# NVIDIA-AI-IOT/redtail

Measured on AMD Instinct MI355X. Metric: stereo pairs/sec, ResNet18-2D 1257x369, higher is better.
Workload: dtype f32

## Files before the change

### redtail_amd/csrc/kernels/common.hip.h

```cpp
#pragma once
#include <hip/hip_runtime.h>
#include <stdint.h>

namespace rt {

typedef float f32x4 __attribute__((ext_vector_type(4)));
typedef float f32x16 __attribute__((ext_vector_type(16)));
typedef _Float16 f16x2 __attribute__((ext_vector_type(2)));
typedef _Float16 f16x4 __attribute__((ext_vector_type(4)));
typedef _Float16 f16x8 __attribute__((ext_vector_type(8)));

constexpr int kWave = 64;

#ifndef RT_WAVES_PER_EU
#define RT_WAVES_PER_EU(n) __attribute__((amdgpu_waves_per_eu(n, n)))
#endif

__host__ __device__ static inline int64_t cdiv(int64_t a, int64_t b) { return (a + b - 1) / b; }
__host__ __device__ static inline int round_up(int a, int b) { return (a + b - 1) / b * b; }

__device__ static __forceinline__ float elu1(float x) { return x > 0.f ? x : expf(x) - 1.f; }
__device__ static __forceinline__ float sigmoid1(float x) { return 1.f / (1.f + expf(-x)); }

template <int ACT>
// ... 15 lines not shown

typedef __amdgpu_buffer_rsrc_t buf_rsrc;
constexpr unsigned kBufOOB = 0x80000000u;
constexpr unsigned kBufSpan = 0x80000000u;
__device__ static __forceinline__ buf_rsrc make_buf(const void* base, bool valid = true) {
    return __builtin_amdgcn_make_buffer_rsrc(const_cast<void*>(base), 0, valid ? kBufSpan : 0u, 0x00020000);
}
__device__ static __forceinline__ float buf_load(buf_rsrc r, unsigned voff, unsigned soff) {
    return __builtin_bit_cast(float, __builtin_amdgcn_raw_buffer_load_b32(r, voff, soff, 0));
}
__device__ static __forceinline__ f32x4 buf_load4(buf_rsrc r, unsigned voff, unsigned soff) {
    return __builtin_bit_cast(f32x4, __builtin_amdgcn_raw_buffer_load_b128(r, voff, soff, 0));
}
typedef float f32x2_t __attribute__((ext_vector_type(2)));
typedef unsigned u32x2_t __attribute__((ext_vector_type(2)));
typedef unsigned u32x4_t __attribute__((ext_vector_type(4)));
__device__ static __forceinline__ f32x2_t buf_load2(buf_rsrc r, unsigned voff, unsigned soff) {
    return __builtin_bit_cast(f32x2_t, __builtin_amdgcn_raw_buffer_load_b64(r, voff, soff, 0));
}
__device__ static __forceinline__ void buf_store2(f32x2_t v, buf_rsrc r, unsigned voff, unsigned soff) {
    __builtin_amdgcn_raw_buffer_store_b64(__builtin_bit_cast(u32x2_t, v), r, voff, soff, 0);
}
__device__ static __forceinline__ void buf_store4(f32x4 v, buf_rsrc r, unsigned voff, unsigned soff) {
    __builtin_amdgcn_raw_buffer_store_b128(__builtin_bit_cast(u32x4_t, v), r, voff + soff, 0u, 0);
}
__device__ static __forceinline__ void buf_store(float v, buf_rsrc r, unsigned voff, unsigned soff) {
    __builtin_amdgcn_raw_buffer_store_b32(__builtin_bit_cast(unsigned, v), r, voff, soff, 0);
}

#ifndef RT_LDS_PTR
#define RT_LDS_PTR(p) ((__attribute__((address_space(3))) void*)(p))
#endif

#ifdef HIPEMU
__device__ static __forceinline__ void wait_vmem() {}
template <int N> __device__ static __forceinline__ void wait_vmem_but() {}
static inline void sload2_i32(const void* base, int off0, int off1, int& a, int& b) {
    a = *reinterpret_cast<const int*>(static_cast<const char*>(base) + off0);
    b = *reinterpret_cast<const int*>(static_cast<const char*>(base) + off1);
}
static inline void sload2_i64(const void* base, int off0, int off1, long long& a, long long& b) {
    a = *reinterpret_cast<const long long*>(static_cast<const char*>(base) + off0);
    b = *reinterpret_cast<const long long*>(static_cast<const char*>(base) + off1);
}
__device__ static __forceinline__ void lds_barrier() { __syncthreads(); }
__device__ static __forceinline__ void wave_lds_sync() { (void)__shfl(0.f, 0); }
__device__ static __forceinline__ unsigned pack_f16(float lo, float hi) {
    return (unsigned)__builtin_bit_cast(unsigned short, (_Float16)lo) | ((unsigned)__builtin_bit_cast(unsigned short, (_Float16)hi) << 16);
}
#else
__device__ static __forceinline__ void sload2_i32(const void* base, int off0, int off1, int& a, int& b) {
    asm volatile("s_load_dword %0, %2, %3\n\ts_load_dword %1, %2, %4\n\ts_waitcnt lgkmcnt(0)" : "=&s"(a), "=&s"(b) : "s"(base), "s"(off0), "s"(off1) : "memory");
}
__device__ static __forceinline__ void sload2_i64(const void* base, int off0, int off1, long long& a, long long& b) {
    asm volatile("s_load_dwordx2 %0, %2, %3\n\ts_load_dwordx2 %1, %2, %4\n\ts_waitcnt lgkmcnt(0)" : "=&s"(a), "=&s"(b) : "s"(base), "s"(off0), "s"(off1) : "memory");
}
__device__ static __forceinline__ void wait_vmem() { asm volatile("s_waitcnt vmcnt(0)" ::: "memory"); }
template <int N> __device__ static __forceinline__ void wait_vmem_but() { asm volatile("s_waitcnt vmcnt(%0)" ::"n"(N) : "memory"); }
__device__ static __forceinline__ void lds_barrier() { asm volatile("s_waitcnt lgkmcnt(0)\n\ts_barrier" ::: "memory"); }
__device__ static __forceinline__ void wave_lds_sync() {
    __builtin_amdgcn_fence(__ATOMIC_RELEASE, "wavefront");
    __builtin_amdgcn_wave_barrier();
    __builtin_amdgcn_fence(__ATOMIC_ACQUIRE, "wavefront");
}
__device__ static __forceinline__ unsigned pack_f16(float lo, float hi) {
    unsigned r;
// ... 38 lines not shown
```

### redtail_amd/csrc/kernels/conv_mfma.hip.h

```cpp
#pragma once
#include <type_traits>
#include "common.hip.h"

namespace rt {

struct ZSlice {
    int pad_y, pad_x;
    int Ho, Wo;
    int ch_row;
    unsigned tap_mask;
    int64_t y_off;
    int64_t w_off;
    int64_t r_off;
    int64_t r_off_il8;
    int64_t y_off_il8;
    int64_t r_off_il4;
};

struct ConvArgs {
    const float* x;
    float* y;
    const float* w;
    const float* bias;
    const float* resid;
    unsigned long long* dbg;
    const float* zeros;
    const ZSlice* zs;
    const int* ch_off;
    int CinPad;
    int Cout;
    int Hi, Wi;
    int x_pitch;
    int Ho, Wo;
    int pad_y, pad_x;
    int nz;
    int tiles_x;
    int act;
    int xcd_order;
    int64_t x_bstride;
    int64_t y_bstride;
    int64_t y_cstride;
    int64_t y_zstride;
    int64_t y_off;
    int y_ystride, y_xstride;
    int64_t r_cstride;
    int64_t r_bstride;
    int r_il8;
    int batch;
    int cin_real;
    int64_t x_cstride;
    const int* ch_shift;
    int w_exact;
    int z_inner;
    int nb_inner;
    int dw_seg, dw_nseg, dw_cpc, dw_ntiles;
    const float* x2;
    int x2_from;
};

#define RT_WG_TILE_NB(p, tile, zi, n, nblk)                                                         \
    int tile = blockIdx.x;                                                                          \
    if ((p).xcd_order) {                           \
        const int nwg_ = gridDim.x, q_ = nwg_ >> 3, r_ = nwg_ & 7;                                  \
        const int xcd_ = blockIdx.x & 7, idx_ = blockIdx.x >> 3;                                    \
        tile = (xcd_ < r_ ? xcd_ * (q_ + 1) : r_ * (q_ + 1) + (xcd_ - r_) * q_) + idx_;             \
    }                                                                                               \
    int nblk = blockIdx.y;                                                                          \
    if ((p).nb_inner > 0) { nblk = tile % (p).nb_inner; tile /= (p).nb_inner; }                     \
    int zi, n;                                                                                      \
    if ((p).z_inner) { zi = tile % (p).nz; tile /= (p).nz; n = blockIdx.z; }                        \
    else { zi = blockIdx.z % (p).nz; n = blockIdx.z / (p).nz; }
#define RT_WG_TILE(p, tile, zi, n) RT_WG_TILE_NB(p, tile, zi, n, nblk_unused_); (void)nblk_unused_;

#ifdef RT_KERNEL_TIMING
#define RT_TSTAMP() do { if (dbgp && tid == 0 && dbi < 16) dbgp[dbi++] = __builtin_amdgcn_s_memtime(); } while (0)
#else
#define RT_TSTAMP() do { } while (0)
#endif

#ifndef RT_ABLATE
#define RT_ABLATE 0
#endif
constexpr bool kAblGather = (RT_ABLATE & 1) != 0;
constexpr bool kAblWLoad = (RT_ABLATE & 2) != 0;
constexpr bool kAblLdsWr = (RT_ABLATE & 4) != 0;
constexpr bool kAblBarrier = (RT_ABLATE & 8) != 0;
constexpr bool kAblResid = (RT_ABLATE & 16) != 0;
constexpr bool kAblStore = (RT_ABLATE & 32) != 0;
constexpr bool kAblLdsRd = (RT_ABLATE & 64) != 0;
constexpr bool kAblXform = (RT_ABLATE & 128) != 0;
// ... 399 lines not shown
```

### redtail_amd/csrc/kernels/conv_rbd.hip.h

```cpp
#pragma once
#include "conv_split.hip.h"

namespace rt {

struct S3RBDCfg {
    static constexpr int NW = 8, NT = 512;
    static constexpr int SW = 30, XCOL = 34, TCOL = 32, STEP = 4;
    static constexpr int RX = 16, RT = 10;
    static constexpr int GXB = XCOL * 32, XROWB = 4 * GXB;
    static constexpr int GTB = TCOL * 32, TROWB = 4 * GTB;
    static constexpr int BSLOTS = STEP * XROWB / 16;
    static constexpr int NPIECE = BSLOTS / 64;
    static constexpr int PPW = (NPIECE + NW - 1) / NW;
    static constexpr int WL_SLOTS = 18 * 64;
    static_assert(BSLOTS % 64 == 0, "a batch is a whole number of DMA pieces");
};

__device__ static __forceinline__ int rbd_swz(int p) { return ((p >> 3) & 1) * 16; }

__device__ static __forceinline__ void rbd_dma16(buf_rsrc rs, void* lds_wave_base, unsigned voff, unsigned soff) {
#ifdef HIPEMU
    __builtin_amdgcn_raw_ptr_buffer_load_lds(rs, lds_wave_base, 16, voff, soff, 0, 0);
#else
    const unsigned m = (unsigned)(uintptr_t)(__attribute__((address_space(3))) char*)(lds_wave_base);
    asm volatile("s_mov_b32 m0, %0\n\ts_nop 0\n\tbuffer_load_dwordx4 %1, %2, %3 offen lds" ::"s"(m), "v"(voff), "s"(rs), "s"(soff) : "memory", "m0");
#endif
}

template <int J>
__device__ static __forceinline__ float rbd_join(unsigned hi2, unsigned lo2, float inv) {
#ifdef HIPEMU
    const _Float16 h = __builtin_bit_cast(_Float16, (unsigned short)(hi2 >> (16 * J))), l = __builtin_bit_cast(_Float16, (unsigned short)(lo2 >> (16 * J)));
    return fmaf((float)l, inv, (float)h);
#else
    float r;
    if (J == 0) asm("v_fma_mix_f32 %0, %1, %2, %3 op_sel:[0,0,0] op_sel_hi:[1,0,1]" : "=v"(r) : "v"(lo2), "v"(inv), "v"(hi2));
    else asm("v_fma_mix_f32 %0, %1, %2, %3 op_sel:[1,0,1] op_sel_hi:[1,0,1]" : "=v"(r) : "v"(lo2), "v"(inv), "v"(hi2));
    return r;
#endif
}

__device__ static __forceinline__ float rbd_elu(float v) { return elu_fast(v); }

#ifndef RT_RBD_PRIO
#define RT_RBD_PRIO 0
#endif
#ifndef RT_RBD_ABL
#define RT_RBD_ABL 0
#endif
#ifndef RT_RBD_PF
#define RT_RBD_PF 1
#endif

template <bool Y_SPLIT>
__global__ void __launch_bounds__(512) RT_WAVES_PER_EU(2) conv_s3rbd_kernel(RBArgs a) {
    using Cfg = S3RBDCfg;
    const ConvArgs& p = a.c;
    constexpr int RX = Cfg::RX, RT = Cfg::RT, GXB = Cfg::GXB, XROWB = Cfg::XROWB, GTB = Cfg::GTB, TROWB = Cfg::TROWB, PPW = Cfg::PPW;

    __shared__ __attribute__((aligned(1024))) char sX[RX * XROWB];
    __shared__ __attribute__((aligned(1024))) char sT[(RT + 2) * TROWB];
// ... 21 lines not shown
        tile = (xcd < r ? xcd * (q + 1) : r * (q + 1) + (xcd - r) * q) + idx;
    }
    const int H = p.Hi, W = p.Wi;
    const int c0 = (tile % p.tiles_x) * Cfg::SW;
    const int y0 = (tile / p.tiles_x) * a.seg;
    const int y1 = y0 + a.seg < H ? y0 + a.seg : H;
    const int t0 = y0 - 1;
    const int n = blockIdx.z;
    const int nstep = (y1 - t0 + 4) / 4 + 1;
    const int last1 = (y1 - t0) / 4;
    const int row_hi = (y1 + 1 < H - 1 ? y1 + 1 : H - 1);

    const buf_rsrc rs_x = make_buf(elem_ptr(p.x, (int64_t)n * p.x_bstride, 4));
    const unsigned gsb_x = (unsigned)p.x_cstride * 32u, rowb_x = (unsigned)p.x_pitch * 32u;
    unsigned xvo[PPW];
    int xnb[PPW];
#pragma unroll
    for (int j = 0; j < PPW; j++) {
        const int k = (wv + 8 * j) * 64 + lane;
        const int r = k / (XROWB / 16), rem = k - r * (XROWB / 16);
        const int g = rem / (GXB / 16), rem2 = rem - g * (GXB / 16);
        const int px = rem2 >> 1, lo = (rem2 & 1) != ((px >> 3) & 1);
        const int ix = c0 - 2 + px;
        const bool valid = wv + 8 * j < Cfg::NPIECE && ix >= 0 && ix < W;
        xvo[j] = valid ? (unsigned)g * gsb_x + (unsigned)(t0 + 1 + r) * rowb_x + (unsigned)ix * 32u + (lo ? 16u : 0u) : kBufOOB;
        const int d = row_hi - (t0 + 1 + r);
        xnb[j] = valid && d >= 0 ? (d >> 2) + 1 : 0;
    }
    auto issue_batch = [&](int b) __attribute__((always_inline)) {
        const unsigned so = (unsigned)(4 * b) * rowb_x;
        char* dst = sX + ((4 * b + 4) & (RX - 1)) * XROWB;
#pragma unroll
        for (int j = 0; j < PPW; j++)
            if (wv + 8 * j < Cfg::NPIECE) rbd_dma16(rs_x, dst + (wv + 8 * j) * 1024, b < xnb[j] ? xvo[j] : kBufOOB, so);
    };

#pragma unroll
    for (int j = 0; j < PPW; j++) {
        if (wv + 8 * j >= Cfg::NPIECE) continue;
        const int r = ((wv + 8 * j) * 64 + lane) / (XROWB / 16);
        const bool ok = xvo[j] != kBufOOB && r >= 2 && t0 - 3 + r >= 0;
        rbd_dma16(rs_x, sX + (wv + 8 * j) * 1024, ok ? xvo[j] - 4u * rowb_x : kBufOOB, 0u);
    }
    issue_batch(0);
    {
        const buf_rsrc rs_w = make_buf(is1 ? a.w1 : p.w);
#pragma unroll
        for (int jj = 0; jj < 9; jj++) {
            const int pw = wr + 4 * jj, t = pw >> 1;
            char* dst = (pw & 1) ? reinterpret_cast<char*>(sWl + (is1 ? 0 : Cfg::WL_SLOTS)) + t * 1024 : sT + (is1 ? 0 : Cfg::WL_SLOTS * 16) + t * 1024;
            rbd_dma16(rs_w, dst, (unsigned)lane * 16u, (unsigned)pw * 1024u);
        }
    }
    f32x16 biasv;
    {
        const float* bsrc = is1 ? a.bias1 : p.bias;
#pragma unroll
        for (int q = 0; q < 4; q++) {
            const f32x4 bv = *reinterpret_cast<const f32x4*>(bsrc + 16 * (q >> 1) + 8 * kg + 4 * (q & 1));
#pragma unroll
            for (int e = 0; e < 4; e++) biasv[4 * q + e] = bv[e];
        }
    }
    RBD_STAMP(1);
    wait_vmem();
#ifndef HIPEMU
    asm volatile("" : "+v"(biasv));
#endif
    __syncthreads();
    f16x8 wh[18];
    {
        const f32x4* whs = reinterpret_cast<const f32x4*>(sT) + (is1 ? 0 : Cfg::WL_SLOTS) + lane;
#pragma unroll
        for (int t = 0; t < 18; t++) wh[t] = __builtin_bit_cast(f16x8, whs[t * 64]);
    }
    __syncthreads();
    RBD_STAMP(2);

    const f32x4* wlp = sWl + (is1 ? 0 : Cfg::WL_SLOTS) + lane;
    int bo_h[3], bo_l[3];
#pragma unroll
    for (int s = 0; s < 3; s++) {
        bo_h[s] = kg * (is1 ? GXB : GTB) + (l31 + s) * 32 + rbd_swz(l31 + s);
        bo_l[s] = bo_h[s] ^ 16;
// ... 185 lines not shown
```

### redtail_amd/csrc/kernels/conv_rbh.hip.h

```cpp
#pragma once
#include "conv_rbd.hip.h"

namespace rt {

struct F16RBDCfg {
    static constexpr int NW = 8, NT = 512;
    static constexpr int SW = 30, XCOL = 36, TCOL = 32, STEP = 4;
    static constexpr int RX = 20, RT = 10;
    static constexpr int GXB = XCOL * 16, XROWB = 4 * GXB;
    static constexpr int GTB = TCOL * 16, TROWB = 4 * GTB;
    static constexpr int BSLOTS = STEP * XROWB / 16;
    static constexpr int NPIECE = BSLOTS / 64;
    static constexpr int PPW = (NPIECE + 3) / 4;
    static constexpr int W_SLOTS = 18 * 64;
    static_assert(BSLOTS % 64 == 0, "a batch is a whole number of DMA pieces");
};

template <int J>
__device__ static __forceinline__ float rbh_add16(unsigned h2, float b) {
#ifdef HIPEMU
    return b + (float)__builtin_bit_cast(_Float16, (unsigned short)(h2 >> (16 * J)));
#else
    float r;
    if (J == 0) asm("v_fma_mix_f32 %0, %1, 1.0, %2 op_sel:[0,0,0] op_sel_hi:[1,0,0]" : "=v"(r) : "v"(h2), "v"(b));
// ... 25 lines not shown
        const int xcd = blockIdx.x & 7, idx = blockIdx.x >> 3;
        tile = (xcd < r ? xcd * (q + 1) : r * (q + 1) + (xcd - r) * q) + idx;
    }
    const int H = p.Hi, W = p.Wi;
    const int c0 = (tile % p.tiles_x) * Cfg::SW;
    const int y0 = (tile / p.tiles_x) * a.seg;
    const int y1 = y0 + a.seg < H ? y0 + a.seg : H;
    const int t0 = y0 - 1;
    const int n = blockIdx.z;
    const int nstep = (y1 - t0 + 4) / 4 + 1;
    const int last1 = (y1 - t0) / 4;
    const int row_hi = (y1 + 1 < H - 1 ? y1 + 1 : H - 1);

    const buf_rsrc rs_x = make_buf(elem_ptr(p.x, (int64_t)n * p.x_bstride, ES));
    const unsigned gsb_x = (unsigned)p.x_cstride * 16u, rowb_x = (unsigned)p.x_pitch * 16u;
    unsigned xvo[PPW];
    int xnb[PPW];
#pragma unroll
    for (int j = 0; j < PPW; j++) {
        const int k = (wr + 4 * j) * 64 + lane;
        const int r = k / (XROWB / 16), rem = k - r * (XROWB / 16);
        const int g = rem / Cfg::XCOL, px = rem - g * Cfg::XCOL;
        const int ix = c0 - 2 + px;
        const bool valid = is1 && wr + 4 * j < Cfg::NPIECE && px < 34 && ix >= 0 && ix < W;
        xvo[j] = valid ? (unsigned)g * gsb_x + (unsigned)(t0 + 1 + r) * rowb_x + (unsigned)ix * 16u : kBufOOB;
        const int d = row_hi - (t0 + 1 + r);
        xnb[j] = valid && d >= 0 ? (d >> 2) + 1 : 0;
    }
    auto issue_batch = [&](int b) __attribute__((always_inline)) {
        const unsigned so = (unsigned)(4 * b) * rowb_x;
        char* dst = sX + ((4 * b + 4) % RX) * XROWB;
#pragma unroll
        for (int j = 0; j < PPW; j++)
            if (wr + 4 * j < Cfg::NPIECE) rbd_dma16(rs_x, dst + (wr + 4 * j) * 1024, b < xnb[j] ? xvo[j] : kBufOOB, so);
    };

    if (is1) {
#pragma unroll
        for (int j = 0; j < PPW; j++) {
            if (wr + 4 * j >= Cfg::NPIECE) continue;
            const int r = ((wr + 4 * j) * 64 + lane) / (XROWB / 16);
            const bool ok = xvo[j] != kBufOOB && r >= 2 && t0 - 3 + r >= 0;
            rbd_dma16(rs_x, sX + (wr + 4 * j) * 1024, ok ? xvo[j] - 4u * rowb_x : kBufOOB, 0u);
        }
        issue_batch(0);
        issue_batch(1);
    }
    {
        const buf_rsrc rs_w = make_buf(is1 ? a.w1 : p.w);
        for (int t = wr; t < 18; t += 4)
            rbd_dma16(rs_w, (is1 ? sT : sX + 12 * XROWB) + t * 1024, (unsigned)lane * 16u, (unsigned)t * 1024u);
    }
    f32x16 biasv;
    {
        const float* bsrc = is1 ? a.bias1 : p.bias;
#pragma unroll
        for (int q = 0; q < 4; q++) {
            const f32x4 bv = *reinterpret_cast<const f32x4*>(bsrc + 16 * (q >> 1) + 8 * kg + 4 * (q & 1));
#pragma unroll
            for (int e = 0; e < 4; e++) biasv[4 * q + e] = bv[e];
        }
    }
    wait_vmem();
#ifndef HIPEMU
    asm volatile("" : "+v"(biasv));
#endif
    __syncthreads();
    f16x8 wh[18];
    {
        const f32x4* whs = reinterpret_cast<const f32x4*>(is1 ? sT : sX + 12 * XROWB) + lane;
#pragma unroll
        for (int t = 0; t < 18; t++) wh[t] = __builtin_bit_cast(f16x8, whs[t * 64]);
    }

    const int bo = kg * (is1 ? GXB : GTB) + l31 * 16;
    constexpr int PF = 1;
    auto contract = [&](auto ring1, int first, f32x16 init) __attribute__((always_inline)) -> f32x16 {
        constexpr bool R1 = decltype(ring1)::value;
        constexpr int NR = R1 ? RX : RT, ROWB = R1 ? XROWB : TROWB, GB = R1 ? GXB : GTB;
        const char* ring = R1 ? sX : sT;
        int so[3];
#pragma unroll
        for (int r = 0; r < 3; r++) {
            const int slot = first + r;
// ... 101 lines not shown
```

### redtail_amd/csrc/kernels/conv_split.hip.h

```cpp
#pragma once
#include <type_traits>
#include "common.hip.h"
#include "conv_mfma.hip.h"

namespace rt {

constexpr float kSplitScale = 2048.f;
constexpr float kSplitInv = 1.f / 2048.f;

struct S3Split {
    f16x4 hi, lo;
};
__device__ static __forceinline__ S3Split s3_split(f32x4 v) {
    S3Split s;
#ifdef HIPEMU
#pragma unroll
    for (int j = 0; j < 4; j++) {
        const _Float16 h = (_Float16)v[j];
        s.hi[j] = h;
        s.lo[j] = (_Float16)((v[j] - (float)h) * kSplitScale);
    }
#else
    unsigned h[2], l[2];
#pragma unroll
// ... 202 lines not shown
    if (dbgp && tid == 0) { dbgp[14] = __builtin_amdgcn_s_memtime(); dbgp[15] = __builtin_amdgcn_s_memrealtime() - rt0; }
#endif
}

}

namespace rt {

template <int KH, int KW, int S, int NW_ = 4>
struct S3Cfg {
    static constexpr int NW = NW_, TY = NW_, TX = 32, CC = 16, TAPS = KH * KW, NT = 64 * NW_;
    static constexpr int PR = (TY - 1) * S + KH, PC = (TX - 1) * S + KW;
    static constexpr int PCH = (PC + 1) / 2;
    static constexpr int PCL = S == 2 ? 2 * PCH : PC;
    static constexpr int NPART = NW / 4;
    static constexpr int NPIX = PR * PC, NKP = ((NPIX + NPART - 1) / NPART + 63) / 64;
    static constexpr int PXB = 80;
    static constexpr int W_SLOTS = TAPS * 2 * 2 * 32;
    static constexpr int NK_W = (W_SLOTS + NT - 1) / NT;
    static constexpr int IN_BYTES = PR * PCL * PXB, GRP_BYTES = IN_BYTES + W_SLOTS * 16;
    static constexpr int KS_MAX = NW_ != 4 ? 1 : (S == 2 ? 2 : 4);
    static constexpr int max_groups(int want) {
        int ks = want < 1 ? 1 : (want > KS_MAX ? KS_MAX : want);
        while (ks > 1 && (ks == 3 || ks * GRP_BYTES < (ks - 1) * NW * 64 * 16 * 4)) ks--;
        return ks;
    }
    static_assert(IN_BYTES % 16 == 0, "weight image alignment");
    static_assert(S == 1 || S == 2, "stride 1 or 2");
};

#ifndef RT_S3_WAVES
#define RT_S3_WAVES(S) ((S) == 2 ? 2 : 4)
#endif
template <int KH, int KW, int S, bool XIL, bool YIL, int NW = 4, typename TIN = float, typename TOUT = float>
__global__ void __launch_bounds__(64 * NW * (S3Cfg<KH, KW, S, NW>::KS_MAX)) RT_WAVES_PER_EU(RT_S3_WAVES(S)) conv_s3_kernel(ConvArgs p) {
    using Cfg = S3Cfg<KH, KW, S, NW>;
    constexpr bool XF16 = std::is_same<TIN, _Float16>::value, YF16 = std::is_same<TOUT, _Float16>::value;
    constexpr unsigned ESX = Io<TIN>::ES, ESY = Io<TOUT>::ES;
    static_assert(!XIL || !XF16, "interleaved fp16 input: conv_f16mma_kernel");
    constexpr int TY = Cfg::TY, TX = Cfg::TX, CC = Cfg::CC, TAPS = Cfg::TAPS, PC = Cfg::PC, PCL = Cfg::PCL, PXB = Cfg::PXB;
    constexpr int NKP = Cfg::NKP, NK_W = Cfg::NK_W, NT = Cfg::NT;

    constexpr int IN_BYTES = Cfg::IN_BYTES, GRP_BYTES = Cfg::GRP_BYTES;
#ifdef HIPEMU
    HIP_DYNAMIC_SHARED(char, smem)
#else
    extern __shared__ __attribute__((aligned(16))) char smem[];
#endif

    const int tid_wg = threadIdx.x;
    const int KS = Cfg::KS_MAX == 1 ? 1 : __builtin_amdgcn_readfirstlane((int)blockDim.x / NT);
    const int kgi = Cfg::KS_MAX == 1 ? 0 : __builtin_amdgcn_readfirstlane(tid_wg / NT);
    const int tid = tid_wg - kgi * NT;
    char* const sIn = smem + kgi * GRP_BYTES;
    f32x4* const sW = reinterpret_cast<f32x4*>(smem + kgi * GRP_BYTES + IN_BYTES);
#ifdef RT_KERNEL_TIMING
    unsigned long long* dbgp = (p.dbg && kgi == 0) ? p.dbg + ((size_t)(blockIdx.z * gridDim.y + blockIdx.y) * gridDim.x + blockIdx.x) * 16 : nullptr;
    int dbi = 0;
    const unsigned long long rt0 = __builtin_amdgcn_s_memrealtime();
#endif
    RT_TSTAMP();
    const int lane = tid & 63;
    const int kg = lane >> 5, l31 = lane & 31;
    const int wv = __builtin_amdgcn_readfirstlane(tid >> 6);

    RT_WG_TILE_NB(p, tile, zi, n, nblk)
// ... 6 lines not shown
    int64_t y_off_il4 = 4 * p.y_off + (int64_t)zi * p.y_zstride, r_off_il4 = y_off_il4;
    unsigned tap_mask = ~0u;
    if (p.zs) {
        const ZSlice z = p.zs[zi];
        pad_y = z.pad_y; pad_x = z.pad_x; Ho = z.Ho; Wo = z.Wo; ch_row = z.ch_row; y_off = z.y_off; w_off = z.w_off;
        r_off = z.r_off; r_off_il8 = z.r_off_il8;
        y_off_il4 = 4 * z.y_off;
        r_off_il4 = z.r_off_il4;
        tap_mask = z.tap_mask;
    }
    const int act = p.act;

    const int sg = wv & 3, spart = wv >> 2;
    const int* __restrict__ tab = p.ch_off + (int64_t)ch_row * p.CinPad + 4 * sg;
    unsigned voff[NKP];
    int lidx[NKP], xcol[NKP];
    const int* __restrict__ shtab = p.ch_shift ? p.ch_shift + (int64_t)ch_row * p.CinPad + 4 * sg : nullptr;
#pragma unroll
    for (int k = 0; k < NKP; k++) {
        const int pidx = spart * (NKP * 64) + lane + 64 * k;
        const int pr = pidx / PC, pc = pidx - pr * PC;
        const int iy = ty0 * S - pad_y + pr, ix = tx0 * S - pad_x + pc;
        const bool own = pidx < Cfg::NPIX && lane + 64 * k < NKP * 64;
        xcol[k] = ix;
        voff[k] = (own && iy >= 0 && iy < p.Hi && ix >= 0 && ix < p.Wi) ? (unsigned)(iy * p.x_pitch + ix) * (XIL ? 16u : ESX) : kBufOOB;
        const int col = S == 2 ? (pc & 1) * Cfg::PCH + (pc >> 1) : pc;
        lidx[k] = own ? (pr * PCL + col) * PXB + sg * 8 : -1;
    }
    const char* __restrict__ wsrc = reinterpret_cast<const char*>(p.w) + (w_off + ((int64_t)nblk * nchunks) * Cfg::W_SLOTS) * 16;
    const buf_rsrc rs_w = make_buf(wsrc);

    f32x4 rin[NKP];
    f32x4 rw[NK_W];
    auto prefetch = [&](int ch) {
        if constexpr (XIL) {
            const int off = tab[ch * CC];
            const int sh = shtab ? shtab[ch * CC] : 0;
            const buf_rsrc rs = make_buf(xb, off >= 0);
#pragma unroll
            for (int k = 0; k < NKP; k++) {
                const unsigned vo = sh == 0 ? voff[k] : ((voff[k] != kBufOOB && xcol[k] >= sh) ? voff[k] - (unsigned)sh * 16u : kBufOOB);
                rin[k] = buf_load4(rs, vo, (unsigned)off * 4u);
            }
        } else {
            const int sh = shtab ? shtab[ch * CC] : 0;
#pragma unroll
            for (int j = 0; j < 4; j++) {
                const int off = tab[ch * CC + j];
                const buf_rsrc rs = make_buf(xb, off >= 0);
#pragma unroll
                for (int k = 0; k < NKP; k++) {
                    const unsigned vo = sh == 0 ? voff[k] : ((voff[k] != kBufOOB && xcol[k] >= sh) ? voff[k] - (unsigned)sh * ESX : kBufOOB);
                    rin[k][j] = Io<TIN>::load(rs, vo, (unsigned)off * ESX);
                }
            }
        }
        const unsigned so = (unsigned)ch * (unsigned)(Cfg::W_SLOTS * 16);
#pragma unroll
        for (int k = 0; k < NK_W; k++) {
            const int idx = tid + NT * k;
            rw[k] = buf_load4(rs_w, idx < Cfg::W_SLOTS ? (unsigned)idx * 16u : kBufOOB, so);
        }
    };
    auto stage_to_lds = [&]() {
#pragma unroll
        for (int k = 0; k < NKP; k++) {
            if (lidx[k] < 0) continue;
            if constexpr (XF16) {
                f16x4 h;
#pragma unroll
                for (int j = 0; j < 4; j++) h[j] = (_Float16)rin[k][j];
                *reinterpret_cast<f16x4*>(sIn + lidx[k]) = h;
            } else {
                const S3Split s = s3_split(rin[k]);
                *reinterpret_cast<f16x4*>(sIn + lidx[k]) = s.hi;
                *reinterpret_cast<f16x4*>(sIn + lidx[k] + 32) = s.lo;
            }
        }
#pragma unroll
        for (int k = 0; k < NK_W; k++) {
            const int idx = tid + NT * k;
            if (idx < Cfg::W_SLOTS) sW[idx] = rw[k];
        }
    };

    const int64_t ybase = (int64_t)n * p.y_bstride + y_off;
    const int64_t rbase = (int64_t)n * p.r_bstride + r_off;
    const int cs32 = (int)p.y_cstride, rs32 = (int)p.r_cstride;
    const int oy = ty0 + wv, ox = tx0 + l31;
    const bool inb = oy < Ho && ox < Wo;
    const bool r_il = p.r_il8 != 0;
    const int cb = nblk * 32;
    f32x4 rr[4];
    if (p.resid != nullptr && kgi == 0) {
        const buf_rsrc rs_r = make_buf(elem_ptr(p.resid, r_il ? (int64_t)n * p.r_bstride + (YF16 ? r_off_il8 : r_off_il4) : rbase, ESY));
        if (r_il && YF16) {
            const unsigned vo = inb ? (unsigned)((oy * p.y_ystride + ox * p.y_xstride) * 8 + 4 * kg) * 2u : kBufOOB;
#pragma unroll
            for (int q = 0; q < 4; q++) {
                const u32x2_t u = __builtin_amdgcn_raw_buffer_load_b64(rs_r, (cb + 8 * q + 4 * kg < p.Cout) ? vo : kBufOOB, (unsigned)((cb + 8 * q) * rs32) * 2u, 0);
#pragma unroll
                for (int e = 0; e < 4; e++) rr[q][e] = (float)__builtin_bit_cast(_Float16, (unsigned short)(u[e >> 1] >> (16 * (e & 1))));
            }
        } else if (r_il) {
            const unsigned vo = inb ? (unsigned)((oy * p.y_ystride + ox * p.y_xstride) * 4 + 4 * kg * rs32) * 4u : kBufOOB;
#pragma unroll
            for (int q = 0; q < 4; q++) rr[q] = buf_load4(rs_r, (cb + 8 * q + 4 * kg < p.Cout) ? vo : kBufOOB, (unsigned)((cb + 8 * q) * rs32) * 4u);
        } else {
            const unsigned vo = inb ? (unsigned)(oy * p.y_ystride + ox * p.y_xstride + 4 * kg * rs32) * ESY : kBufOOB;
#pragma unroll
            for (int q = 0; q < 4; q++)
#pragma unroll
                for (int e = 0; e < 4; e++)
                    rr[q][e] = Io<TOUT>::load(rs_r, (cb + 8 * q + 4 * kg + e < p.Cout) ? vo : kBufOOB, (unsigned)((cb + 8 * q + e) * rs32) * ESY);
        }
    } else {
#pragma unroll
        for (int q = 0; q < 4; q++) rr[q] = f32x4{0.f, 0.f, 0.f, 0.f};
    }

    f32x16 acc_m, acc_c;
#pragma unroll
    for (int r = 0; r < 16; r++) { acc_m[r] = 0.f; acc_c[r] = 0.f; }
    const int a_off = kg * 32 + l31;
    const bool w_exact = p.w_exact != 0;
    const int b_off = (wv * S * PCL + l31) * PXB + kg * 16;
    auto compute = [&]() {
#pragma unroll
        for (int t = 0; t < TAPS; t++) {
            if (!((tap_mask >> t) & 1u)) continue;
            const int r = t / KW, s = t % KW;
            const int col = S == 2 ? (s & 1) * Cfg::PCH + (s >> 1) : s;
            const char* bp = sIn + b_off + (r * PCL + col) * PXB;
            const f16x8 bh = *reinterpret_cast<const f16x8*>(bp);
            const f16x8 ah = __builtin_bit_cast(f16x8, sW[a_off + (t * 2 + 0) * 64]);
            acc_m = __builtin_amdgcn_mfma_f32_32x32x16_f16(ah, bh, acc_m, 0, 0, 0);
            if (!w_exact) {
                const f16x8 al = __builtin_bit_cast(f16x8, sW[a_off + (t * 2 + 1) * 64]);
                acc_c = __builtin_amdgcn_mfma_f32_32x32x16_f16(al, bh, acc_c, 0, 0, 0);
            }
            if constexpr (!XF16) {
                const f16x8 bl = *reinterpret_cast<const f16x8*>(bp + 32);
                acc_c = __builtin_amdgcn_mfma_f32_32x32x16_f16(ah, bl, acc_c, 0, 0, 0);
            }
        }
    };

    if (kgi < nchunks) prefetch(kgi);
    RT_TSTAMP();
    for (int ch = kgi; ch < nchunks + kgi; ch += KS) {
        const bool mine = KS == 1 || ch < nchunks;
        if (ch != kgi) __syncthreads();
        if (mine) stage_to_lds();
        __syncthreads();
        RT_TSTAMP();
        if (ch + KS < nchunks) prefetch(ch + KS);
        if (mine) compute();
        RT_TSTAMP();
    }

#pragma unroll
    for (int r = 0; r < 16; r++) acc_m[r] = fmaf(acc_c[r], kSplitInv, acc_m[r]);
    if (KS > 1) {
        f32x4* const red = reinterpret_cast<f32x4*>(smem);
        __syncthreads();
        if (kgi > 0) {
#pragma unroll
            for (int q = 0; q < 4; q++)
                red[(((kgi - 1) * NW + wv) * 4 + q) * 64 + lane] = f32x4{acc_m[4 * q], acc_m[4 * q + 1], acc_m[4 * q + 2], acc_m[4 * q + 3]};
        }
        __syncthreads();
        if (kgi > 0) return;
        for (int g = 1; g < KS; g++)
#pragma unroll
            for (int q = 0; q < 4; q++) {
                const f32x4 v = red[(((g - 1) * NW + wv) * 4 + q) * 64 + lane];
#pragma unroll
                for (int e = 0; e < 4; e++) acc_m[4 * q + e] += v[e];
            }
    }

    const buf_rsrc rs_y = make_buf(elem_ptr(p.y, (YIL && !YF16) ? (int64_t)n * p.y_bstride + y_off_il4 : ybase, ESY));
    auto epilogue = [&](auto ACT) {
#pragma unroll
        for (int q = 0; q < 4; q++) {
            const f32x4 bv = *reinterpret_cast<const f32x4*>(p.bias + cb + 8 * q + 4 * kg);
            f32x4 o;
#pragma unroll
            for (int e = 0; e < 4; e++)
                o[e] = apply_act_fast(acc_m[4 * q + e] + (bv[e] + rr[q][e]), decltype(ACT)::value);
            if constexpr (YIL && YF16) {
                const unsigned vo = (inb && cb + 8 * q + 4 * kg < p.Cout) ? (unsigned)((oy * p.y_ystride + ox * p.y_xstride) * 8 + 4 * kg) * 2u : kBufOOB;
                u32x2_t w2;
#pragma unroll
                for (int e = 0; e < 2; e++)
                    w2[e] = (unsigned)__builtin_bit_cast(unsigned short, (_Float16)o[2 * e]) | ((unsigned)__builtin_bit_cast(unsigned short, (_Float16)o[2 * e + 1]) << 16);
                __builtin_amdgcn_raw_buffer_store_b64(w2, rs_y, vo, (unsigned)((cb + 8 * q) * cs32) * 2u, 0);
            } else if constexpr (YIL) {
                const unsigned vo = (inb && cb + 8 * q + 4 * kg < p.Cout) ? (unsigned)((oy * p.y_ystride + ox * p.y_xstride) * 4 + 4 * kg * cs32) * 4u : kBufOOB;
                buf_store4(o, rs_y, vo, (unsigned)((cb + 8 * q) * cs32) * 4u);
            } else {
                const unsigned vo = inb ? (unsigned)(oy * p.y_ystride + ox * p.y_xstride + 4 * kg * cs32) * ESY : kBufOOB;
#pragma unroll
                for (int e = 0; e < 4; e++)
                    Io<TOUT>::store(o[e], rs_y, (cb + 8 * q + 4 * kg + e < p.Cout) ? vo : kBufOOB, (unsigned)((cb + 8 * q + e) * cs32) * ESY);
            }
        }
    };
    if (act == 1) epilogue(std::integral_constant<int, 1>{});
    else if (act == 2) epilogue(std::integral_constant<int, 2>{});
    else epilogue(std::integral_constant<int, 0>{});
    RT_TSTAMP();
#ifdef RT_KERNEL_TIMING
    __builtin_amdgcn_s_waitcnt(0);
    if (dbgp && tid == 0) { dbgp[14] = __builtin_amdgcn_s_memtime(); dbgp[15] = __builtin_amdgcn_s_memrealtime() - rt0; }
#endif
}

}
// ... 365 lines not shown
```

### redtail_amd/csrc/rt_capi.hip

```cpp
#include <hip/hip_runtime.h>

#include <algorithm>
#include <atomic>
#include <cstdarg>
#include <cstdio>
#include <cstdlib>
#include <cstring>
#include <string>
#include <map>
#include <mutex>
#include <vector>

#include "../../include/rt_stereo.h"
#if defined(__HIP_DEVICE_COMPILE__) && !defined(RT_BUILT_NO_SLP)
#error "rt_capi.hip must be compiled with -fno-slp-vectorize -DRT_BUILT_NO_SLP (redtail_amd/build.py: DEVICE_FLAGS)"
#endif
#include "kernels/common.hip.h"
#include "kernels/conv_mfma.hip.h"
#include "kernels/conv_wino.hip.h"
#include "kernels/deconv3d_small.hip.h"
#include "kernels/imgproc.hip.h"
#include "kernels/conv_f16.hip.h"
#include "kernels/conv_f16_first.hip.h"
#include "kernels/conv_f16r4.hip.h"
// ... 923 lines not shown
                    const int k = 3 * sx + c, h = k / 8, e = k % 8;
                    const size_t blk = (size_t)(co / 32) * rt::S3FirstCfg::W_SLOTS * 8;
                    packed[blk + ((((size_t)r * 2 + 0) * 2 + h) * 32 + co % 32) * 8 + e] = hi;
                    packed[blk + ((((size_t)r * 2 + 1) * 2 + h) * 32 + co % 32) * 8 + e] = lo;
                }
    if (sc.w_dev) (void)hipFree(sc.w_dev);
    sc.w_dev = nullptr;
    RT_HIP(hipMalloc((void**)&sc.w_dev, packed.size() * 2));
    RT_HIP(hipMemcpy(sc.w_dev, packed.data(), packed.size() * 2, hipMemcpyHostToDevice));
    sc.s3first = 1; sc.s3p = 0; sc.split3 = 0; sc.wino = 0;
    sc.NBW = 1; sc.TXW = 1; sc.TY = sc.NW = 4;
    return 0;
}

template <bool Z, int PAT>
bool drop_structural_zeros(std::vector<float>& packed) {
    using Taps = rt::SmallTaps<Z, PAT>;
    constexpr int NJ = Taps::NJ;
    if (env_int("RT_NO_SMALL_SPARSE", 0) != 0) return false;
    const size_t rows = packed.size() / (NJ * NJ);
    for (size_t r = 0; r < rows; r++)
        for (int f = 0; f < NJ; f++)
            for (int j = 0; j < NJ; j++)
                if (!Taps::valid(f, j) && packed[(r * NJ + f) * NJ + j] != 0.f) return false;
    std::vector<float> dense(rows * Taps::NV);
    for (size_t r = 0; r < rows; r++)
        for (int f = 0; f < NJ; f++)
            for (int j = 0; j < NJ; j++)
                if (Taps::valid(f, j)) dense[r * Taps::NV + Taps::index(f, j)] = packed[(r * NJ + f) * NJ + j];
    packed.swap(dense);
    return true;
}

template <typename T> constexpr const char* type_tag() { return sizeof(T) == 2 ? "f16" : "f32"; }
template <int KH, int KW, int S, bool XIL, bool YIL, int NW = 4, typename TIN = float, typename TOUT = float>
void launch_s3(dim3 grid, int ks, int64_t per_cu, hipStream_t st, const rt::ConvArgs& a, int trace = 0) {
    using Cfg = rt::S3Cfg<KH, KW, S, NW>;
    ks = Cfg::max_groups(ks);
    while (ks > 1 && std::min<int64_t>(per_cu, 4) * ks * Cfg::GRP_BYTES > 160 * 1024) ks = Cfg::max_groups(ks - 1);
    if (trace)
        fprintf(stderr, "[rt] conv_s3<%d,%d,%d,%d,%d,%d,%s,%s> r%d grid %u x %u x %u ks %d\n", KH, KW, S, (int)XIL, (int)YIL, NW, type_tag<TIN>(),
                type_tag<TOUT>(), a.r_il8, grid.x, grid.y, grid.z, ks);
#ifndef HIPEMU
    static std::atomic<unsigned long long> done{0};
    int dev = 0;
    if (hipGetDevice(&dev) == hipSuccess && dev >= 0 && dev < 64 && !((done.load(std::memory_order_acquire) >> dev) & 1ull)) {
        (void)hipFuncSetAttribute(reinterpret_cast<const void*>(&rt::conv_s3_kernel<KH, KW, S, XIL, YIL, NW, TIN, TOUT>),
                                  hipFuncAttributeMaxDynamicSharedMemorySize, Cfg::KS_MAX * Cfg::GRP_BYTES);
        done.fetch_or(1ull << dev, std::memory_order_release);
    }
#endif
    hipLaunchKernelGGL((rt::conv_s3_kernel<KH, KW, S, XIL, YIL, NW, TIN, TOUT>), grid, dim3(64 * NW * ks), (size_t)ks * Cfg::GRP_BYTES, st, a);
}

int device_cus() {
    static std::atomic<int> cus[64];
    int dev = 0;
    if (hipGetDevice(&dev) != hipSuccess || dev < 0 || dev >= 64) return 256;
    int n = cus[dev].load(std::memory_order_relaxed);
    if (!n) {
        hipDeviceProp_t prop;
        n = (hipGetDeviceProperties(&prop, dev) == hipSuccess && prop.multiProcessorCount > 0) ? prop.multiProcessorCount : 256;
        cus[dev].store(n, std::memory_order_relaxed);
    }
    return n;
}

std::vector<float> to_f32(const void* w, size_t n, int dtype) {
    std::vector<float> out(n);
    if (dtype == RT_F16) {
        const char* h = static_cast<const char*>(w);
        for (size_t i = 0; i < n; i++) {
            _Float16 v;
            std::memcpy(&v, h + 2 * i, 2);
            out[i] = (float)v;
        }
    } else {
        std::memcpy(out.data(), w, n * sizeof(float));
    }
    return out;
}

template <int KH, int KW, int S, int NBW, int CC>
int launch_window(const SubConv& sc, const rt::ConvArgs& a, dim3 grid, hipStream_t st) {
#define RT_TILE(ty, txw, nw, wlds)                                                                        \
// ... 1420 lines not shown
                    const int seg_len = (int)rt::cdiv(a.Mz, nseg);
                    nseg = (int)rt::cdiv(a.Mz, seg_len);
                    RT_REQUIRE(rowpairs <= 65535, "rt_conv_enqueue: grid limit exceeded");
                    dim3 gw((unsigned)(rt::cdiv(groups, 4) * nseg), (unsigned)rowpairs, (unsigned)batch);
                    if (plan->opt_trace) fprintf(stderr, "[rt] deconv3d_s2_ilw<0> grid %u x %u x %u segments %d x %d\n", gw.x, gw.y, gw.z, nseg, seg_len);
                    hipLaunchKernelGGL(rt::deconv3d_s2_ilw_kernel<0>, gw, dim3(256), 0, S(s), a, seg_len, nseg);
                } else {
                    dim3 g2((unsigned)(rt::cdiv(groups, 4 * rt::kSmallIlIters) * a.Mz), (unsigned)rowpairs, (unsigned)batch);
                    if (plan->opt_trace) fprintf(stderr, "[rt] deconv3d_s2_il grid %u x %u x %u\n", g2.x, g2.y, g2.z);
                    hipLaunchKernelGGL(rt::deconv3d_s2_il_kernel, g2, dim3(256), 0, S(s), a);
                }
            } else if (sc.small3d == 1 && !sc.x_f16 && sc.x_il8) {
                RT_REQUIRE(sc.small_il_dev && sc.small_il_f32, "rt_conv_enqueue: interleaved fp32 input without its weight operands (rt_conv_plan_set_layouts)");
                a.w = static_cast<const float*>(sc.small_il_dev);
                const int groups = (int)rt::cdiv((a.Wx + 1) / 2, 16);
                RT_REQUIRE(batch <= 65535, "rt_conv_enqueue: grid limit exceeded");
                dim3 g2((unsigned)(rt::cdiv(groups, 4 * rt::kSmallIlIters) * a.Mz), (unsigned)rt::cdiv((a.Hx + 1) / 2, 2), (unsigned)batch);
                if (plan->opt_trace) fprintf(stderr, "[rt] deconv3d_s2_il4 grid %u x %u x %u\n", g2.x, g2.y, g2.z);
                hipLaunchKernelGGL(rt::deconv3d_s2_il4_kernel, g2, dim3(256), 0, S(s), a);
            } else if (sc.small3d == 1 && sc.x_f16) {
                if (a.C == 1) hipLaunchKernelGGL((rt::deconv3d_s2_small_kernel<1, true, _Float16, float>), grid, dim3(256), 0, S(s), a);
                else hipLaunchKernelGGL((rt::deconv3d_s2_small_kernel<2, true, _Float16, float>), grid, dim3(256), 0, S(s), a);
            } else if (sc.small3d == 2) {
                if (a.C == 1) hipLaunchKernelGGL((rt::deconv3d_s2_small_kernel<1, false>), grid, dim3(256), 0, S(s), a);
                else hipLaunchKernelGGL((rt::deconv3d_s2_small_kernel<2, false>), grid, dim3(256), 0, S(s), a);
            } else {
                if (a.C == 1) hipLaunchKernelGGL((rt::deconv3d_s2_small_kernel<1, true>), grid, dim3(256), 0, S(s), a);
                else hipLaunchKernelGGL((rt::deconv3d_s2_small_kernel<2, true>), grid, dim3(256), 0, S(s), a);
            }
            RT_LAUNCH_CHECK("deconv3d_s2_small_kernel");
            continue;
        }
        rt::ConvArgs a;
        a.z_inner = 0; a.nb_inner = 0;
        a.x = static_cast<const float*>(x);
        a.x2 = static_cast<const float*>(tl_twin_x2); a.x2_from = tl_twin_from;
        a.y = static_cast<float*>(y);
        a.w = sc.w_dev;
        a.bias = plan->bias_dev;
        a.zeros = plan->zeros_dev;
        a.dbg = nullptr;
#ifdef RT_KERNEL_TIMING
        if (const char* e = getenv("RT_DBG_PTR")) a.dbg = (unsigned long long*)strtoull(e, nullptr, 0);
#endif
        a.resid = plan->has_resid ? static_cast<const float*>(residual) : nullptr;
        a.ch_off = sc.choff_dev;
        a.ch_shift = sc.shift_dev;
        a.w_exact = plan->w_f16;
        a.zs = sc.zs_dev;
        a.CinPad = sc.CinPad; a.Cout = sc.Cout;
        a.Hi = sc.Hi; a.Wi = sc.Wi; a.Ho = sc.Ho; a.Wo = sc.Wo;
        a.x_pitch = sc.x_pitch ? sc.x_pitch : sc.Wi;
        a.pad_y = sc.pad_y; a.pad_x = sc.pad_x; a.nz = sc.nz;
        a.tiles_x = (int)rt::cdiv(sc.Wo, 32 * sc.TXW);
        a.act = plan->act;
        a.xcd_order = plan->opt_xcd;
        a.x_bstride = plan->x_bstride; a.y_bstride = plan->y_bstride;
        a.y_cstride = sc.y_cstride; a.y_zstride = sc.y_zstride; a.y_off = sc.y_off;
        if (plan->is_conv3d && !plan->c3d_dchw && sc.y_il8) a.y_zstride = 8 * sc.y_zstride;
        a.y_ystride = sc.y_ystride; a.y_xstride = sc.y_xstride;
        a.r_cstride = sc.r_cstride ? sc.r_cstride : sc.y_cstride;
        a.r_bstride = plan->r_bstride ? plan->r_bstride : plan->y_bstride;
        a.r_il8 = sc.r_il8;
        a.batch = batch; a.cin_real = sc.cin_real; a.x_cstride = (int64_t)sc.Hi * a.x_pitch;
        if (sc.dp4 && sc.split3) {
            a.tiles_x = (int)rt::cdiv(sc.Wi, 32);
            const int tiles = a.tiles_x * (int)rt::cdiv(sc.Hi, 4), nblk = (int)rt::cdiv(sc.Cout, 32);
// ... 580 lines not shown
```

Baseline: 2724.

## Double-buffer LDS in conv_s3 with weight DMA and software-pipelined tap fetch

When conv_s3 runs with a single group (ks==1), it now keeps two LDS images. Weights for the next chunk are DMA'd straight into LDS with buffer_load...lds, and activations are staged into the alternate buffer while the current chunk computes. This removes one barrier per chunk and the register round-trip for weights. It also prefetches the next tap's operands ahead of the MFMAs, hoists the bias loads, and moves the LDS DMA helper into a shared header. In exchange it doubles LDS per workgroup, which can lower occupancy, and it is gated by an env knob and by an LDS budget check.

```diff
diff --git a/redtail_amd/csrc/kernels/common.hip.h b/redtail_amd/csrc/kernels/common.hip.h
--- a/redtail_amd/csrc/kernels/common.hip.h
+++ b/redtail_amd/csrc/kernels/common.hip.h
@@ -71,6 +71,15 @@
 #define RT_LDS_PTR(p) ((__attribute__((address_space(3))) void*)(p))
 #endif
 
+__device__ static __forceinline__ void lds_dma16(buf_rsrc rs, void* lds_wave_base, unsigned voff, unsigned soff) {
+#ifdef HIPEMU
+    __builtin_amdgcn_raw_ptr_buffer_load_lds(rs, lds_wave_base, 16, voff, soff, 0, 0);
+#else
+    const unsigned m = (unsigned)(uintptr_t)(__attribute__((address_space(3))) char*)(lds_wave_base);
+    asm volatile("s_mov_b32 m0, %0\n\ts_nop 0\n\tbuffer_load_dwordx4 %1, %2, %3 offen lds" ::"s"(m), "v"(voff), "s"(rs), "s"(soff) : "memory", "m0");
+#endif
+}
+
 #ifdef HIPEMU
 __device__ static __forceinline__ void wait_vmem() {}
 template <int N> __device__ static __forceinline__ void wait_vmem_but() {}
diff --git a/redtail_amd/csrc/kernels/conv_mfma.hip.h b/redtail_amd/csrc/kernels/conv_mfma.hip.h
--- a/redtail_amd/csrc/kernels/conv_mfma.hip.h
+++ b/redtail_amd/csrc/kernels/conv_mfma.hip.h
@@ -56,6 +56,7 @@
     int dw_seg, dw_nseg, dw_cpc, dw_ntiles;
     const float* x2;
     int x2_from;
+    int s3_dbl;
 };
 
 #define RT_WG_TILE_NB(p, tile, zi, n, nblk)                                                         \
diff --git a/redtail_amd/csrc/kernels/conv_rbd.hip.h b/redtail_amd/csrc/kernels/conv_rbd.hip.h
--- a/redtail_amd/csrc/kernels/conv_rbd.hip.h
+++ b/redtail_amd/csrc/kernels/conv_rbd.hip.h
@@ -18,15 +18,6 @@
 
 __device__ static __forceinline__ int rbd_swz(int p) { return ((p >> 3) & 1) * 16; }
 
-__device__ static __forceinline__ void rbd_dma16(buf_rsrc rs, void* lds_wave_base, unsigned voff, unsigned soff) {
-#ifdef HIPEMU
-    __builtin_amdgcn_raw_ptr_buffer_load_lds(rs, lds_wave_base, 16, voff, soff, 0, 0);
-#else
-    const unsigned m = (unsigned)(uintptr_t)(__attribute__((address_space(3))) char*)(lds_wave_base);
-    asm volatile("s_mov_b32 m0, %0\n\ts_nop 0\n\tbuffer_load_dwordx4 %1, %2, %3 offen lds" ::"s"(m), "v"(voff), "s"(rs), "s"(soff) : "memory", "m0");
-#endif
-}
-
 template <int J>
 __device__ static __forceinline__ float rbd_join(unsigned hi2, unsigned lo2, float inv) {
 #ifdef HIPEMU
@@ -114,7 +105,7 @@
         char* dst = sX + ((4 * b + 4) & (RX - 1)) * XROWB;
 #pragma unroll
         for (int j = 0; j < PPW; j++)
-            if (wv + 8 * j < Cfg::NPIECE) rbd_dma16(rs_x, dst + (wv + 8 * j) * 1024, b < xnb[j] ? xvo[j] : kBufOOB, so);
+            if (wv + 8 * j < Cfg::NPIECE) lds_dma16(rs_x, dst + (wv + 8 * j) * 1024, b < xnb[j] ? xvo[j] : kBufOOB, so);
     };
 
 #pragma unroll
@@ -122,7 +113,7 @@
         if (wv + 8 * j >= Cfg::NPIECE) continue;
         const int r = ((wv + 8 * j) * 64 + lane) / (XROWB / 16);
         const bool ok = xvo[j] != kBufOOB && r >= 2 && t0 - 3 + r >= 0;
-        rbd_dma16(rs_x, sX + (wv + 8 * j) * 1024, ok ? xvo[j] - 4u * rowb_x : kBufOOB, 0u);
+        lds_dma16(rs_x, sX + (wv + 8 * j) * 1024, ok ? xvo[j] - 4u * rowb_x : kBufOOB, 0u);
     }
     issue_batch(0);
     {
@@ -131,7 +122,7 @@
         for (int jj = 0; jj < 9; jj++) {
             const int pw = wr + 4 * jj, t = pw >> 1;
             char* dst = (pw & 1) ? reinterpret_cast<char*>(sWl + (is1 ? 0 : Cfg::WL_SLOTS)) + t * 1024 : sT + (is1 ? 0 : Cfg::WL_SLOTS * 16) + t * 1024;
-            rbd_dma16(rs_w, dst, (unsigned)lane * 16u, (unsigned)pw * 1024u);
+            lds_dma16(rs_w, dst, (unsigned)lane * 16u, (unsigned)pw * 1024u);
         }
     }
     f32x16 biasv;
diff --git a/redtail_amd/csrc/kernels/conv_rbh.hip.h b/redtail_amd/csrc/kernels/conv_rbh.hip.h
--- a/redtail_amd/csrc/kernels/conv_rbh.hip.h
+++ b/redtail_amd/csrc/kernels/conv_rbh.hip.h
@@ -81,7 +81,7 @@
         char* dst = sX + ((4 * b + 4) % RX) * XROWB;
 #pragma unroll
         for (int j = 0; j < PPW; j++)
-            if (wr + 4 * j < Cfg::NPIECE) rbd_dma16(rs_x, dst + (wr + 4 * j) * 1024, b < xnb[j] ? xvo[j] : kBufOOB, so);
+            if (wr + 4 * j < Cfg::NPIECE) lds_dma16(rs_x, dst + (wr + 4 * j) * 1024, b < xnb[j] ? xvo[j] : kBufOOB, so);
     };
 
     if (is1) {
@@ -90,7 +90,7 @@
             if (wr + 4 * j >= Cfg::NPIECE) continue;
             const int r = ((wr + 4 * j) * 64 + lane) / (XROWB / 16);
             const bool ok = xvo[j] != kBufOOB && r >= 2 && t0 - 3 + r >= 0;
-            rbd_dma16(rs_x, sX + (wr + 4 * j) * 1024, ok ? xvo[j] - 4u * rowb_x : kBufOOB, 0u);
+            lds_dma16(rs_x, sX + (wr + 4 * j) * 1024, ok ? xvo[j] - 4u * rowb_x : kBufOOB, 0u);
         }
         issue_batch(0);
         issue_batch(1);
@@ -98,7 +98,7 @@
     {
         const buf_rsrc rs_w = make_buf(is1 ? a.w1 : p.w);
         for (int t = wr; t < 18; t += 4)
-            rbd_dma16(rs_w, (is1 ? sT : sX + 12 * XROWB) + t * 1024, (unsigned)lane * 16u, (unsigned)t * 1024u);
+            lds_dma16(rs_w, (is1 ? sT : sX + 12 * XROWB) + t * 1024, (unsigned)lane * 16u, (unsigned)t * 1024u);
     }
     f32x16 biasv;
     {
diff --git a/redtail_amd/csrc/kernels/conv_split.hip.h b/redtail_amd/csrc/kernels/conv_split.hip.h
--- a/redtail_amd/csrc/kernels/conv_split.hip.h
+++ b/redtail_amd/csrc/kernels/conv_split.hip.h
@@ -258,6 +258,11 @@
 #ifndef RT_S3_WAVES
 #define RT_S3_WAVES(S) ((S) == 2 ? 2 : 4)
 #endif
+template <int KH, int KW, int S, bool XIL, bool YIL, int NW, typename TIN, typename TOUT>
+constexpr bool s3_two_image() {
+    return NW == 4 && (!(KH == 3 && KW == 3 && S == 1) || (XIL && YIL && sizeof(TIN) == 4 && sizeof(TOUT) == 4));
+}
+
 template <int KH, int KW, int S, bool XIL, bool YIL, int NW = 4, typename TIN = float, typename TOUT = float>
 __global__ void __launch_bounds__(64 * NW * (S3Cfg<KH, KW, S, NW>::KS_MAX)) RT_WAVES_PER_EU(RT_S3_WAVES(S)) conv_s3_kernel(ConvArgs p) {
     using Cfg = S3Cfg<KH, KW, S, NW>;
@@ -330,7 +335,7 @@
 
     f32x4 rin[NKP];
     f32x4 rw[NK_W];
-    auto prefetch = [&](int ch) {
+    auto prefetch_x = [&](int ch) {
         if constexpr (XIL) {
             const int off = tab[ch * CC];
             const int sh = shtab ? shtab[ch * CC] : 0;
@@ -353,6 +358,9 @@
                 }
             }
         }
+    };
+    auto prefetch = [&](int ch) {
+        prefetch_x(ch);
         const unsigned so = (unsigned)ch * (unsigned)(Cfg::W_SLOTS * 16);
 #pragma unroll
         for (int k = 0; k < NK_W; k++) {
@@ -360,7 +368,7 @@
             rw[k] = buf_load4(rs_w, idx < Cfg::W_SLOTS ? (unsigned)idx * 16u : kBufOOB, so);
         }
     };
-    auto stage_to_lds = [&]() {
+    auto stage_x = [&](char* img) {
 #pragma unroll
         for (int k = 0; k < NKP; k++) {
             if (lidx[k] < 0) continue;
@@ -368,17 +376,30 @@
                 f16x4 h;
 #pragma unroll
                 for (int j = 0; j < 4; j++) h[j] = (_Float16)rin[k][j];
-                *reinterpret_cast<f16x4*>(sIn + lidx[k]) = h;
+                *reinterpret_cast<f16x4*>(img + lidx[k]) = h;
             } else {
                 const S3Split s = s3_split(rin[k]);
-                *reinterpret_cast<f16x4*>(sIn + lidx[k]) = s.hi;
-                *reinterpret_cast<f16x4*>(sIn + lidx[k] + 32) = s.lo;
-            }
-        }
+                *reinterpret_cast<f16x4*>(img + lidx[k]) = s.hi;
+                *reinterpret_cast<f16x4*>(img + lidx[k] + 32) = s.lo;
+            }
+        }
+    };
+    auto stage_to_lds = [&]() {
+        stage_x(sIn);
 #pragma unroll
         for (int k = 0; k < NK_W; k++) {
             const int idx = tid + NT * k;
             if (idx < Cfg::W_SLOTS) sW[idx] = rw[k];
+        }
+    };
+    constexpr int W_PIECES = Cfg::W_SLOTS / 64;
+    static_assert(Cfg::W_SLOTS % 64 == 0, "the weights of a chunk are whole DMA pieces");
+    auto dma_w = [&](int ch, char* img) {
+        const unsigned so = (unsigned)ch * (unsigned)(Cfg::W_SLOTS * 16);
+#pragma unroll
+        for (int j = 0; j < (W_PIECES + NW - 1) / NW; j++) {
+            const int pc = wv + NW * j;
+            if (pc < W_PIECES) lds_dma16(rs_w, img + IN_BYTES + pc * 1024, (unsigned)lane * 16u, so + (unsigned)pc * 1024u);
         }
     };
 
@@ -443,18 +464,83 @@
             }
         }
     };
-
-    if (kgi < nchunks) prefetch(kgi);
-    RT_TSTAMP();
-    for (int ch = kgi; ch < nchunks + kgi; ch += KS) {
-        const bool mine = KS == 1 || ch < nchunks;
-        if (ch != kgi) __syncthreads();
-        if (mine) stage_to_lds();
-        __syncthreads();
+    struct Ops {
+        f16x8 ah, al, bh, bl;
+    };
+    auto fetch = [&](const char* img, int t) {
+        const int r = t / KW, s = t % KW;
+        const int col = S == 2 ? (s & 1) * Cfg::PCH + (s >> 1) : s;
+        const char* bp = img + b_off + (r * PCL + col) * PXB;
+        const f32x4* w = reinterpret_cast<const f32x4*>(img + IN_BYTES);
+        Ops o;
+        o.bh = *reinterpret_cast<const f16x8*>(bp);
+        o.ah = __builtin_bit_cast(f16x8, w[a_off + (t * 2 + 0) * 64]);
+        o.al = __builtin_bit_cast(f16x8, w[a_off + (t * 2 + 1) * 64]);
+        if constexpr (!XF16) o.bl = *reinterpret_cast<const f16x8*>(bp + 32);
+        else o.bl = o.bh;
+        return o;
+    };
+    auto compute_ahead = [&](const char* img) {
+        Ops cur = fetch(img, 0);
+#pragma unroll
+        for (int t = 0; t < TAPS; t++) {
+            Ops nxt = cur;
+            if (t + 1 < TAPS) nxt = fetch(img, t + 1);
+            if ((tap_mask >> t) & 1u) {
+                acc_m = __builtin_amdgcn_mfma_f32_32x32x16_f16(cur.ah, cur.bh, acc_m, 0, 0, 0);
+                if (!w_exact) acc_c = __builtin_amdgcn_mfma_f32_32x32x16_f16(cur.al, cur.bh, acc_c, 0, 0, 0);
+                if constexpr (!XF16) acc_c = __builtin_amdgcn_mfma_f32_32x32x16_f16(cur.ah, cur.bl, acc_c, 0, 0, 0);
+            }
+            cur = nxt;
+        }
+    };
+    f32x4 bq[4];
+    auto load_bias = [&]() {
+#pragma unroll
+        for (int q = 0; q < 4; q++) bq[q] = *reinterpret_cast<const f32x4*>(p.bias + cb + 8 * q + 4 * kg);
+    };
+
+    if (s3_two_image<KH, KW, S, XIL, YIL, NW, TIN, TOUT>() && KS == 1 && p.s3_dbl) {
+        char* const img0 = smem;
+        char* const img1 = smem + GRP_BYTES;
+        prefetch_x(0);
+        dma_w(0, img0);
         RT_TSTAMP();
-        if (ch + KS < nchunks) prefetch(ch + KS);
-        if (mine) compute();
+        stage_x(img0);
+        wait_vmem();
+        if (nchunks > 1) {
+            prefetch_x(1);
+            dma_w(1, img1);
+        }
+        for (int ch = 0; ch < nchunks; ch++) {
+            char* const cur = (ch & 1) ? img1 : img0;
+            char* const nxt = (ch & 1) ? img0 : img1;
+            __syncthreads();
+            RT_TSTAMP();
+            if (ch > 0 && ch + 1 < nchunks) dma_w(ch + 1, nxt);
+            compute_ahead(cur);
+            if (ch + 1 < nchunks) {
+                stage_x(nxt);
+                wait_vmem();
+                if (ch + 2 < nchunks) prefetch_x(ch + 2);
+            }
+            RT_TSTAMP();
+        }
+        load_bias();
+    } else {
+        if (kgi < nchunks) prefetch(kgi);
         RT_TSTAMP();
+        for (int ch = kgi; ch < nchunks + kgi; ch += KS) {
+            const bool mine = KS == 1 || ch < nchunks;
+            if (ch != kgi) __syncthreads();
+            if (mine) stage_to_lds();
+            __syncthreads();
+            RT_TSTAMP();
+            if (ch + KS < nchunks) prefetch(ch + KS);
+            if (mine) compute();
+            RT_TSTAMP();
+        }
+        load_bias();
     }
 
 #pragma unroll
@@ -482,7 +568,7 @@
     auto epilogue = [&](auto ACT) {
 #pragma unroll
         for (int q = 0; q < 4; q++) {
-            const f32x4 bv = *reinterpret_cast<const f32x4*>(p.bias + cb + 8 * q + 4 * kg);
+            const f32x4 bv = bq[q];
             f32x4 o;
 #pragma unroll
             for (int e = 0; e < 4; e++)
diff --git a/redtail_amd/csrc/rt_capi.hip b/redtail_amd/csrc/rt_capi.hip
--- a/redtail_amd/csrc/rt_capi.hip
+++ b/redtail_amd/csrc/rt_capi.hip
@@ -979,12 +979,20 @@
     return true;
 }
 
+bool s3_dbl_knob() {
+    static const bool on = env_int("RT_S3_DBL", 1) != 0;
+    return on;
+}
+
 template <typename T> constexpr const char* type_tag() { return sizeof(T) == 2 ? "f16" : "f32"; }
 template <int KH, int KW, int S, bool XIL, bool YIL, int NW = 4, typename TIN = float, typename TOUT = float>
 void launch_s3(dim3 grid, int ks, int64_t per_cu, hipStream_t st, const rt::ConvArgs& a, int trace = 0) {
     using Cfg = rt::S3Cfg<KH, KW, S, NW>;
     ks = Cfg::max_groups(ks);
     while (ks > 1 && std::min<int64_t>(per_cu, 4) * ks * Cfg::GRP_BYTES > 160 * 1024) ks = Cfg::max_groups(ks - 1);
+    rt::ConvArgs b = a;
+    b.s3_dbl = rt::s3_two_image<KH, KW, S, XIL, YIL, NW, TIN, TOUT>() && ks == 1 && s3_dbl_knob() && a.CinPad >= 2 * Cfg::CC &&
+               std::min<int64_t>(per_cu, 4) * 2 * Cfg::GRP_BYTES <= 160 * 1024;
     if (trace)
         fprintf(stderr, "[rt] conv_s3<%d,%d,%d,%d,%d,%d,%s,%s> r%d grid %u x %u x %u ks %d\n", KH, KW, S, (int)XIL, (int)YIL, NW, type_tag<TIN>(),
                 type_tag<TOUT>(), a.r_il8, grid.x, grid.y, grid.z, ks);
@@ -993,11 +1001,12 @@
     int dev = 0;
     if (hipGetDevice(&dev) == hipSuccess && dev >= 0 && dev < 64 && !((done.load(std::memory_order_acquire) >> dev) & 1ull)) {
         (void)hipFuncSetAttribute(reinterpret_cast<const void*>(&rt::conv_s3_kernel<KH, KW, S, XIL, YIL, NW, TIN, TOUT>),
-                                  hipFuncAttributeMaxDynamicSharedMemorySize, Cfg::KS_MAX * Cfg::GRP_BYTES);
+                                  hipFuncAttributeMaxDynamicSharedMemorySize, std::max(Cfg::KS_MAX, 2) * Cfg::GRP_BYTES);
         done.fetch_or(1ull << dev, std::memory_order_release);
     }
 #endif
-    hipLaunchKernelGGL((rt::conv_s3_kernel<KH, KW, S, XIL, YIL, NW, TIN, TOUT>), grid, dim3(64 * NW * ks), (size_t)ks * Cfg::GRP_BYTES, st, a);
+    hipLaunchKernelGGL((rt::conv_s3_kernel<KH, KW, S, XIL, YIL, NW, TIN, TOUT>), grid, dim3(64 * NW * ks), (size_t)(b.s3_dbl ? 2 : ks) * Cfg::GRP_BYTES,
+                       st, b);
 }
 
 int device_cus() {
@@ -2484,7 +2493,7 @@
             continue;
         }
         rt::ConvArgs a;
-        a.z_inner = 0; a.nb_inner = 0;
+        a.z_inner = 0; a.nb_inner = 0; a.s3_dbl = 0;
         a.x = static_cast<const float*>(x);
         a.x2 = static_cast<const float*>(tl_twin_x2); a.x2_from = tl_twin_from;
         a.y = static_cast<float*>(y);
```

New measurement: 2694 (median of 6 runs). 0.989x the previous value.
